# YamaneKoyo/mri-to-speech

Measured on AMD Instinct MI355X. Metric: rtMRI frames/s end-to-end (256x256 frames -> 64-bin mel -> 11413 Hz wav), higher is better.
Workload: dtype bf16x3; 1 GPU; e2e rtMRI->wav, 64 clips x 30 frames per GPU at 256x256 (configs[3] per-GPU share); clips_per_gpu=64, frames_per_clip=30, global_batch_clips=64, hw=256, parallelism=dp1, chunk=1920

## Files before the change

### mri-to-speech_amd/csrc/ir_ws.hip

```cpp
#include <algorithm>
#include <cstdlib>
#include <type_traits>
#include <vector>

#include "kernels.hpp"
#include "lds_dma.hpp"
#include "prof.hpp"

namespace m2s {
namespace {

constexpr int WS_SL = 32;
constexpr int WS_BR = 8;
constexpr int WS_NP = 8;
constexpr int WS_NC = 8;
constexpr int WS_UMAX = 3;

__device__ __forceinline__ int hx_of(int r) { return ((r & 3) << 2) | swz_f((r >> 2) & 3); }

struct WsLayout {
  int XR, TROWS, x_bytes, tile_bytes, w_bytes, total;
};

__host__ __device__ inline int ws_cpp(int cs_in) { return (cs_in * 2 + 255) / 256 * 16; }
// ... 228 lines not shown
      TR(f, 13);
      bump(pdone_p);
      if (JOINT) {
        wait_pd_tf(f, d2);
        return;
      }
      if (f + 1 < T) wait_ge(pdone_p, NPC * (unsigned)(f + 1));
      TR(f, 14);
      if (f + 2 < T) issue_w(f + 2, d2);
    }
  };
  auto produce = [&](int f, Step d, Step d2) {
    const int r0 = d.band * WS_BR, br = min(WS_BR, H - r0), xr0 = max(r0 - 1, 0), xr1 = min(r0 + WS_BR + 1, H);
    const int PB = (xr1 - xr0) * W, nunit = 2 * ((PB + 15) / 16);
    const char* wb = wbuf + (f & 1) * KS * 4096;
    const int hxl = hx_of(r16);
    static_assert(WS_NP % 2 == 0, "unit -> channel tile");
    const int wrow = (wave & 1) * 16 + r16;
    const int wo = wrow * 64 + ((g ^ swz_f((wrow >> 2) & 3)) << 4);
    const int nu = nunit > wave ? (nunit - wave + WS_NP - 1) / WS_NP : 0;
    char* tb = tiles + (f & 1) * 8 * PLT;
    const int trow0 = xr0 - r0 + 1;
    const float4 bb = *reinterpret_cast<const float4*>(bpl + (f & 1) * 32 + (wave & 1) * 16 + 4 * g);
    auto units = [&](auto nuc) {
      constexpr int NU = decltype(nuc)::value;
      f32x4 acc[NU];
#pragma unroll
      for (int k = 0; k < NU; ++k) acc[k] = f32x4{0.f, 0.f, 0.f, 0.f};
      constexpr int D = !IRWS_PF_DEEP ? 2 : NU == 1 ? 4 : NU == 2 ? 3 : 2;
      bf16x8 ah[D], al[D], bh[D][NU], bl[D][NU];
      auto load = [&](int ks, int bsel) {
        const int Lh = ks * 4 + g, Ll = CPP + ks * 4 + g;
        const int ph = ((Lh & ~15) | ((Lh & 15) ^ hxl)) << 4, pl = ((Ll & ~15) | ((Ll & 15) ^ hxl)) << 4;
        ah[bsel] = *reinterpret_cast<const bf16x8*>(wb + ks * 4096 + wo);
        al[bsel] = *reinterpret_cast<const bf16x8*>(wb + ks * 4096 + 2048 + wo);
#pragma unroll
        for (int k = 0; k < NU; ++k) {
          const char* xr = xs + (((wave + WS_NP * k) >> 1) * 16 + r16) * XP;
          bh[bsel][k] = *reinterpret_cast<const bf16x8*>(xr + ph);
          bl[bsel][k] = *reinterpret_cast<const bf16x8*>(xr + pl);
        }
      };
#pragma unroll
      for (int ks = 0; ks < D - 1 && ks < KS; ++ks) load(ks, ks);
#pragma unroll
      for (int ks = 0; ks < KS; ++ks) {
        const int c = ks % D;
        if (ks + D - 1 < KS) load(ks + D - 1, (ks + D - 1) % D);
        __builtin_amdgcn_sched_barrier(0);
#pragma unroll
        for (int k = 0; k < NU; ++k) {
          acc[k] = __builtin_amdgcn_mfma_f32_16x16x32_bf16(al[c], bh[c][k], acc[k], 0, 0, 0);
          acc[k] = __builtin_amdgcn_mfma_f32_16x16x32_bf16(ah[c], bl[c][k], acc[k], 0, 0, 0);
          acc[k] = __builtin_amdgcn_mfma_f32_16x16x32_bf16(ah[c], bh[c][k], acc[k], 0, 0, 0);
        }
      }
      TR(f, 6);
      after_mfma(f, d2);
      TR(f, 8);
      if (!JOINT && f >= 2) wait_all(tfree, (unsigned)(f - 1));
      TR(f, 9);
#pragma unroll
      for (int k = 0; k < NU; ++k) {
        const int u = wave + WS_NP * k, nt = u & 1, m = (u >> 1) * 16 + r16;
        if (m < PB) {
          const int ti = (m / W + trow0) * WT + (m % W) + 1;
          *reinterpret_cast<float4*>(tb + (nt * 4 + g) * PLT + ti * 16) =
              make_float4(silu(acc[k][0] + bb.x), silu(acc[k][1] + bb.y), silu(acc[k][2] + bb.z), silu(acc[k][3] + bb.w));
        }
      }
    };
    static_assert(WS_UMAX == 3, "unit counts 1..3");
    if (nu == 3) units(std::integral_constant<int, 3>());
    else if (nu == 2) units(std::integral_constant<int, 2>());
    else if (nu == 1) units(std::integral_constant<int, 1>());
    else {
      after_mfma(f, d2);
      if (!JOINT && f >= 2) wait_all(tfree, (unsigned)(f - 1));
    }
    if (tid < 8 * W) {
      const int pl = tid / W, c = tid - pl * W;
      const float4 z = make_float4(0.f, 0.f, 0.f, 0.f);
      if (r0 == 0) *reinterpret_cast<float4*>(tb + pl * PLT + (c + 1) * 16) = z;
      if (r0 + br == H) *reinterpret_cast<float4*>(tb + pl * PLT + ((br + 1) * WT + c + 1) * 16) = z;
    }
  };

  const int ct = tid - 64 * WS_NP, cw = ct >> 6, cg = ct & 7, cpl = ct >> 3;
  int cpo = cpl, toff0 = ((cpl / W) * WT + cpl % W) * 16;
  if constexpr (S == 2) {
    const int k = cpl >> 2, i = cpl & 3, c0 = (k >> 1) + 4 * (k & 1);
    const int oy = 2 * (k & 1) + (i & 1), ox = (((i & 1) ? c0 + 6 : c0) + 4 * (i >> 1)) & 7;
    cpo = oy * OWS + ox;
    toff0 = ((2 * oy - pad_t + 1) * WT + 2 * ox - pad_l + 1) * 16;
  }
  auto consume = [&](int f, Step d) {
    const int c0 = d.sl * WS_SL, r0 = d.band * WS_BR, br = min(WS_BR, H - r0);
    float s[4] = {0.f, 0.f, 0.f, 0.f};
    TR(f, 4);
    const uint32_t pbase = (uint32_t)(d.img * PO + (r0 / S) * OWS);
    const uint32_t yoffb = __builtin_amdgcn_readfirstlane(4u * (uint32_t)c0) + (fm32 ? 16u : 8u) * (uint32_t)cg +
                           pbase * (4u * (uint32_t)cs_mid);
    const uint32_t yoff0 = yoffb + (uint32_t)cpo * (4u * (uint32_t)cs_mid);
    const float* wd = wdl + (f % 3) * 320 + 4 * cg;
    float w[9][4], b[4];
#pragma unroll
    for (int t = 0; t < 9; ++t) {
      const float4 v = *reinterpret_cast<const float4*>(wd + t * 32);
      w[t][0] = v.x; w[t][1] = v.y; w[t][2] = v.z; w[t][3] = v.w;
    }
    {
      const float4 v = *reinterpret_cast<const float4*>(wd + 288);
      b[0] = v.x; b[1] = v.y; b[2] = v.z; b[3] = v.w;
    }
    const char* tpl = tiles + (f & 1) * 8 * PLT + cg * PLT;
    auto pixel = [&](int k) {
      const char* tp = tpl + toff0 + k * (64 / W) * WT * 16;
      float a[4] = {b[0], b[1], b[2], b[3]};
#pragma unroll
      for (int t = 0; t < 9; ++t) {
        const float4 u = *reinterpret_cast<const float4*>(tp + ((t / 3) * WT + (t % 3)) * 16);
        a[0] += w[t][0] * u.x;
        a[1] += w[t][1] * u.y;
        a[2] += w[t][2] * u.z;
        a[3] += w[t][3] * u.w;
        if (t == 5) asm volatile("" ::: "memory");
      }
#pragma unroll
      for (int j = 0; j < 4; ++j) {
        a[j] = silu(a[j]);
        s[j] += a[j];
      }
      char* u = reinterpret_cast<char*>(y) + (yoff0 + (uint32_t)k * 256u * (uint32_t)cs_mid);
      if (fm32) {
        *reinterpret_cast<float4*>(u) = make_float4(a[0], a[1], a[2], a[3]);
      } else {
        uint2 hi, lo;
        split4(a, hi, lo);
        *reinterpret_cast<uint2*>(u) = hi;
        *reinterpret_cast<uint2*>(u + 64) = lo;
      }
    };
    auto pixel_pair = [&]() {
      const int pa = cpl >> 4, pc = cpl & 15;
      const char* tp = tpl + ((2 * pa) * WT + pc) * 16;
      float a0[4] = {b[0], b[1], b[2], b[3]}, a1[4] = {b[0], b[1], b[2], b[3]};
#pragma unroll
      for (int ry = 0; ry < 4; ++ry) {
#pragma unroll
        for (int rx = 0; rx < 3; ++rx) {
          const float4 u = *reinterpret_cast<const float4*>(tp + (ry * WT + rx) * 16);
          if (ry < 3) {
            const int t = ry * 3 + rx;
            a0[0] += w[t][0] * u.x; a0[1] += w[t][1] * u.y; a0[2] += w[t][2] * u.z; a0[3] += w[t][3] * u.w;
          }
          if (ry > 0) {
            const int t = (ry - 1) * 3 + rx;
            a1[0] += w[t][0] * u.x; a1[1] += w[t][1] * u.y; a1[2] += w[t][2] * u.z; a1[3] += w[t][3] * u.w;
          }
        }
        if (ry == 1) asm volatile("" ::: "memory");
      }
      const uint32_t po = (uint32_t)(32 * pa + pc);
      auto out = [&](float* a, uint32_t pos) {
#pragma unroll
        for (int j = 0; j < 4; ++j) {
          a[j] = silu(a[j]);
          s[j] += a[j];
        }
        char* u = reinterpret_cast<char*>(y) + (yoffb + pos * (4u * (uint32_t)cs_mid));
        if (fm32) {
          *reinterpret_cast<float4*>(u) = make_float4(a[0], a[1], a[2], a[3]);
        } else {
          uint2 hi, lo;
          split4(a, hi, lo);
          *reinterpret_cast<uint2*>(u) = hi;
          *reinterpret_cast<uint2*>(u + 64) = lo;
        }
      };
      out(a0, po);
      out(a1, po + 16u);
    };
    if constexpr (S == 2) {
      if (cpl < OPB) pixel(0);
    } else if (IRWS_PAIR && W == 16 && br == WS_BR) {
      pixel_pair();
    } else if (br == WS_BR) {
#pragma unroll
      for (int k = 0; k < WS_PXL; ++k) pixel(k);
    } else {
#pragma unroll
      for (int k = 0; k < WS_PXL; ++k)
        if (cpl + 64 * k < br * W) pixel(k);
    }
    TR(f, 5);
    bump(tfree + cw);
    TR(f, 10);
#pragma unroll
    for (int j = 0; j < 4; ++j) {
      s[j] += __builtin_bit_cast(float, __builtin_amdgcn_update_dpp(0, __builtin_bit_cast(int, s[j]), 0x128, 0xF, 0xF, false));
      const auto q = __builtin_amdgcn_permlane16_swap(__float_as_uint(s[j]), __float_as_uint(s[j]), false, false);
      s[j] = __uint_as_float(q[0]) + __uint_as_float(q[1]);
      const auto r = __builtin_amdgcn_permlane32_swap(__float_as_uint(s[j]), __float_as_uint(s[j]), false, false);
      s[j] = __uint_as_float(r[0]) + __uint_as_float(r[1]);
    }
    TR(f, 11);
    const int sc = 4 * (lane & 7) + ((lane >> 3) & 3);
    {
      const int j = (lane >> 3) & 3;
      const float v = j == 0 ? s[0] : j == 1 ? s[1] : j == 2 ? s[2] : s[3];
      if (lane < WS_SL && !(__builtin_fabsf(v) < 2147483648.0f))
        asm volatile("ds_write_b32 %0, %1" ::"v"((uint32_t)(uintptr_t)(sq_nan + d.sl)), "v"(1u) : "memory");
      if (lane < WS_SL)
        __hip_atomic_fetch_add(sq + c0 + sc, (unsigned long long)(long long)(__builtin_fabsf(v) < 2147483648.0f ? v * 4294967296.0f : 0.f),
                               __ATOMIC_RELAXED, __HIP_MEMORY_SCOPE_WORKGROUP);
    }
    unsigned arrived = 0;
    if (lane == 0) arrived = __hip_atomic_fetch_add(sq_n + d.sl, 1u, __ATOMIC_ACQ_REL, __HIP_MEMORY_SCOPE_WORKGROUP);
    if (__builtin_amdgcn_readfirstlane(arrived) == (unsigned)(NB * WS_NC - 1) && lane < WS_SL) {
      const unsigned long long t = __hip_atomic_exchange(sq + c0 + sc, 0ull, __ATOMIC_RELAXED, __HIP_MEMORY_SCOPE_WORKGROUP);
      const float m = __fmaf_rn((float)(unsigned)t, 2.3283064365386963e-10f, (float)(int)(t >> 32)) / (float)PO;
      act_st<sp_t>(reinterpret_cast<sp_t*>(se_mean), d.img, cs_mid, c0 + sc, (*poison || sq_nan[d.sl]) ? __builtin_nanf("") : m);
      if (lane == 0) {
        sq_n[d.sl] = 0u;
        sq_nan[d.sl] = 0u;
      }
    }
  };

  __syncthreads();
  if (prod) {
    __builtin_amdgcn_s_setprio(2);
    Step cur = first_step(blockIdx.x);
    if (T > 0) issue_w(0, cur);
    if (T > 1) issue_w(1, next_step(cur));
    if (TAPS_AHEAD && T > 0 && tap_wave) issue_wd(0, cur);
    if (T > 0) {
      wait_vm_le((T > 1 ? npw : 0) + (TAPS_AHEAD && tap_wave ? 1 : 0));
      bump(wrdy_p);
      if (!HAND_END) wait_ge(wrdy_p, NPC);
    }
    static_assert(4 * KS <= 4 * WS_NP, "pieces per wave");
    int bands = 0;
    for (int i = 0; i < T; ++i) {
      const Step nxt = next_step(cur), nxt2 = next_step(nxt);
      TR(i, 0);
      if (cur.sl == cur.lo) {
        if (i > 0) {
          wait_ge(pdone_p, NPC * (unsigned)i);
          if (par) wait_ge(pw ? ctr + 0 : ctr + 5, NPC * (unsigned)i);
        }
        issue_x(cur.img, cur.band);
        wait_vm<0>();
        bump(xrdy);
        wait_ge(xrdy, (unsigned)(WS_NP * ++bands));
      }
      TR(i, 1);
      if (!TAPS_AHEAD && tap_wave) {
        if (i >= 3) wait_all(tfree, (unsigned)(i - 2));
        issue_wd(i, cur);
      }
      if (HAND_END) wait_ge(wrdy_p, NPC * (unsigned)(i + 1));
      TR(i, 2);
      produce(i, cur, nxt2);
      if (HAND_END) {
        wait_vm<0>();
        asm volatile("s_waitcnt lgkmcnt(0)" ::: "memory");
        if (lane == 0) {
          asm volatile("ds_add_u32 %0, %1" ::"v"((uint32_t)(uintptr_t)wrdy_p), "v"(1u) : "memory");
          asm volatile("ds_add_u32 %0, %1" ::"v"((uint32_t)(uintptr_t)tfull), "v"(1u) : "memory");
        }
        TR(i, 12);
        const bool nw = i + 2 < T, nt = TAPS_AHEAD && tap_wave && i + 1 < T;
        if (nw || nt) {
          wait_ge(pdone_p, NPC * (unsigned)(i + 1));
          if (nw) issue_w(i + 2, nxt2);
          if (nt) issue_wd(i + 1, nxt);
        }
      } else {
        if (tap_wave) {
          const bool nt = TAPS_AHEAD && i + 1 < T;
          if (nt) issue_wd(i + 1, nxt);
          wait_vm_le((i + 2 < T ? npw : 0) + (nt ? 1 : 0));
        }
        bump(tfull);
        TR(i, 12);
      }
      TR(i, 3);
      cur = nxt;
    }
  } else {
    Step cur = first_step(blockIdx.x);
    for (int i = 0; i < T; ++i) {
      wait_ge(tfull, (unsigned)(WS_NP * (i + 1)));
      consume(i, cur);
      TR(i, 7);
      cur = next_step(cur);
    }
  }
}

#include "ir_ws_wave.hpp"

constexpr bool ws_wave_shape(int W, int S) { return W == 16 && S == 1; }
template <int W, int KS, int S>
__global__ void __launch_bounds__(ws_wave_shape(W, S) ? 64 * WV_NW : 64 * (WS_NP + WS_NC), 1)
    ir_ws_kernel(const bf16_t* __restrict__ x, int N, int H, int cs_mid, const bf16_t* __restrict__ wpw,
                 const float* __restrict__ bpw, const float* __restrict__ wdw, const float* __restrict__ bdw,
                 bf16_t* __restrict__ y, bf16_t* __restrict__ se_mean, unsigned long long* __restrict__ trace,
                 unsigned spin_max, unsigned* __restrict__ err, int pad_t, int pad_l, int fm32, int n_full, int parts) {
  if constexpr (ws_wave_shape(W, S)) ir_ws_wave16<KS>(x, N, H, cs_mid, wpw, bpw, wdw, bdw, y, se_mean, fm32, n_full, parts);
  else ir_ws_handoff<W, KS, S>(x, N, H, cs_mid, wpw, bpw, wdw, bdw, y, se_mean, trace, spin_max, err, pad_t, pad_l, fm32, n_full, parts);
}
template <int W, int KS, int S, int HANDOFF>
__global__ void __launch_bounds__(64 * (WS_NP + WS_NC), 1)
    ir_ws_kernel(const bf16_t* __restrict__ x, int N, int H, int cs_mid, const bf16_t* __restrict__ wpw,
                 const float* __restrict__ bpw, const float* __restrict__ wdw, const float* __restrict__ bdw,
                 bf16_t* __restrict__ y, bf16_t* __restrict__ se_mean, unsigned long long* __restrict__ trace,
                 unsigned spin_max, unsigned* __restrict__ err, int pad_t, int pad_l, int fm32, int n_full, int parts) {
  static_assert(HANDOFF == 1, "the handed-off form");
  ir_ws_handoff<W, KS, S>(x, N, H, cs_mid, wpw, bpw, wdw, bdw, y, se_mean, trace, spin_max, err, pad_t, pad_l, fm32, n_full, parts);
}

#ifdef IRWS_TRACE
static void dump_trace(unsigned long long* tr, hipStream_t s, const char* tag) {
  static int calls = 0;
  if (++calls > 40) return;
  std::vector<unsigned long long> h(64 * 2 * 16 * 64);
  M2S_HIP(hipStreamSynchronize(s));
  M2S_HIP(hipMemcpy(h.data(), tr, h.size() * 8, hipMemcpyDeviceToHost));
  auto at = [&](int i, int c, int k, int w = 0) { return (long long)h[((i * 2 + c) * 16 + k) * 64 + w]; };
  fprintf(stderr, "TRACE %s:", tag);
  for (int i = 2; i < 12; ++i)
    fprintf(stderr, " [P x %lld wr %lld mfma %lld tf %lld epi %lld hand %lld | C wait %lld px %lld bump %lld shf %lld at %lld]",
            at(i, 0, 1) - at(i, 0, 0), at(i, 0, 2) - at(i, 0, 1), at(i, 0, 6) - at(i, 0, 2), at(i, 0, 9) - at(i, 0, 6),
            at(i, 0, 12) - at(i, 0, 9), at(i, 0, 3) - at(i, 0, 12), at(i, 1, 4) - at(i - 1, 1, 7), at(i, 1, 5) - at(i, 1, 4),
            at(i, 1, 10) - at(i, 1, 5), at(i, 1, 11) - at(i, 1, 10), at(i, 1, 7) - at(i, 1, 11));
  fprintf(stderr, "\n");
  fprintf(stderr, "TRACEW %s:", tag);
  for (int i = 2; i < 4; ++i) {
    fprintf(stderr, " [s%d", i);
    for (int w = 0; w < 8; ++w) {
      fprintf(stderr, " w%d", w);
      for (int k : {0, 2, 6, 9, 12, 3}) fprintf(stderr, "%c%lld", k ? '/' : ' ', at(i, 0, k, w) - at(i, 0, 0));
    }
    fprintf(stderr, "]");
  }
  fprintf(stderr, "\n");
  fprintf(stderr, "TRACEC %s:", tag);
  for (int i = 4; i < 7; ++i) {
    fprintf(stderr, " [s%d P0 mfma_end %lld vm0 %lld pdone %lld after %lld tf %lld tfull %lld |", i, at(i, 0, 6) - at(i, 0, 0),
            at(i, 0, 13) - at(i, 0, 0), at(i, 0, 14) - at(i, 0, 0), at(i, 0, 8) - at(i, 0, 0), at(i, 0, 9) - at(i, 0, 0),
            at(i, 0, 12) - at(i, 0, 0));
    for (int j = i - 2; j <= i; ++j) {
      fprintf(stderr, " c%d:", j);
      for (int w = 0; w < 8; ++w)
        fprintf(stderr, " %lld/%lld/%lld", at(j, 1, 4, w) - at(i, 0, 0), at(j, 1, 10, w) - at(i, 0, 0), at(j, 1, 7, w) - at(i, 0, 0));
    }
    fprintf(stderr, "]");
  }
  fprintf(stderr, "\n");
  M2S_HIP(hipMemset(tr, 0, h.size() * 8));
}
#endif

}

bool ir_ws_s2_supported(int H, int W, int cs_in, int kp, int cs_mid, int OH, int OW, int pad_t, int pad_l) {
  return H == 16 && W == 16 && OH == 8 && OW == 8 && pad_t >= 0 && pad_t <= 1 && pad_l >= 0 && pad_l <= 1 &&
         ir_ws_supported(H, W, cs_in, kp, cs_mid) && ws_layout(H, W, cs_in, cs_mid, 2).total <= 160 * 1024;
}

bool ir_ws_supported(int H, int W, int cs_in, int kp, int cs_mid) {
  if (!((W == 8 && (kp == 128 || kp == 224)) || (W == 16 && kp == 128)) || H < 1 || H > 64 || cs_in != kp) return false;
  if (cs_mid % WS_SL != 0 || cs_mid < 3 * WS_SL) return false;
  const WsLayout L = ws_layout(H, W, cs_in, cs_mid);
  const int cpr = 2 * ws_cpp(cs_in);
  return L.total <= 160 * 1024 && (L.XR * W * cpr) % 64 == 0 && L.XR * W * cpr / 64 / WS_NP + 1 <= 60 &&
         2 * ((L.XR * W + 15) / 16) <= WS_NP * WS_UMAX;
}

void launch_ir_ws(const void* x, int N, int H, int W, int cs_in, int kp, int cs_mid, const void* wpw, const float* bpw,
                  const float* wdw, const float* bdw, void* y, void* se_mean, double flops, double bytes,
                  hipStream_t s, AsyncReport rep, int stride, int OH, int OW, int pad_t, int pad_l, double spill,
                  bool fm32, int forced_parts, bool handoff) {
  M2S_CHECK(stride == 1 ? ir_ws_supported(H, W, cs_in, kp, cs_mid)
                        : stride == 2 && ir_ws_s2_supported(H, W, cs_in, kp, cs_mid, OH, OW, pad_t, pad_l),
            "ir_ws: unsupported shape");
  M2S_CHECK(N > 0, "ir_ws: no images");
  M2S_CHECK((double)N * H * W * cs_mid * 4.0 < 4294967296.0, "ir_ws: output map too large for 32-bit offsets");
  const WsLayout L = ws_layout(H, W, cs_in, cs_mid, stride);
  const int n_cu = device_cus();
  const dim3 grid(std::min(N, n_cu));
  const int G = (int)grid.x, NSl = cs_mid / WS_SL;
  const int n_full = N / G * G, rem = N - n_full;
  int parts = rem > 0 ? std::max(1, (G + rem / 2) / rem) : 1;
  parts = std::max(1, std::min(parts, NSl / 3));
  if (forced_parts > 0) parts = std::min(forced_parts, std::max(1, NSl / 3));
#ifdef IRWS_TRACE
  static unsigned long long* tr = [] {
    unsigned long long* p = nullptr;
    if (getenv("M2S_IR_WS_TRACE")) M2S_HIP(hipMalloc(&p, 64 * 2 * 16 * 64 * 8));
    return p;
  }();
#define M2S_IRWS_DUMP(tag) \
  if (tr) dump_trace(tr, s, tag);
#else
  unsigned long long* tr = nullptr;
#define M2S_IRWS_DUMP(tag)
#endif
  const bf16_t* xb = static_cast<const bf16_t*>(x);
  const bf16_t* wb = static_cast<const bf16_t*>(wpw);
  bf16_t* yb = static_cast<bf16_t*>(y);
  bf16_t* mb = static_cast<bf16_t*>(se_mean);
  const bool wave_form = ws_wave_shape(W, stride) && H <= 16 && !handoff;
#define M2S_IRWS_GO(KERNEL_, THREADS_, LDS_, NAME_)                                                     \
  {                                                                                                     \
    allow_lds(reinterpret_cast<const void*>(&KERNEL_));                                                 \
    ProfScope ps(NAME_, flops, bytes, s, spill);                                                        \
    hipLaunchKernelGGL((KERNEL_), grid, dim3(THREADS_), LDS_, s, xb, N, H, cs_mid, wb, bpw, wdw, bdw, yb, mb, tr, \
                       rep.spin_max, rep.err, pad_t, pad_l, fm32 ? 1 : 0, n_full, parts);               \
    M2S_IRWS_DUMP(NAME_)                                                                                \
    M2S_HIP(hipGetLastError());                                                                         \
    return;                                                                                             \
  }
  if (ws_wave_shape(W, stride) && kp == 128) {
    if (wave_form) M2S_IRWS_GO((ir_ws_kernel<16, 4, 1>), 64 * WV_NW, WV_NW * 1024 + H * W * 2 * ws_cpp(cs_in) * 16, "ir_ws_kernel<16, 4, 1>")
    M2S_IRWS_GO((ir_ws_kernel<16, 4, 1, 1>), 64 * (WS_NP + WS_NC), L.total, "ir_ws_kernel<16, 4, 1, 1>")
  }
#define M2S_IRWS(W_, KS_, S_, NAME_)                                                                    \
  if (W == W_ && kp == KS_ * 32 && stride == S_) M2S_IRWS_GO((ir_ws_kernel<W_, KS_, S_>), 64 * (WS_NP + WS_NC), L.total, NAME_)
  M2S_IRWS(8, 4, 1, "ir_ws_kernel<8, 4, 1>") M2S_IRWS(8, 7, 1, "ir_ws_kernel<8, 7, 1>")
  M2S_IRWS(16, 4, 2, "ir_ws_kernel<16, 4, 2>")
#undef M2S_IRWS_GO
#undef M2S_IRWS
#undef M2S_IRWS_DUMP
  M2S_CHECK(false, "ir_ws: no variant for this shape");
}

}
```

### mri-to-speech_amd/csrc/ir_ws_wave.hpp

```cpp
#pragma once


#ifndef IRWS_WAVE_ABL
#define IRWS_WAVE_ABL 0
#endif
constexpr int WV_NW = 8;
constexpr int WV_GC = 16;
constexpr int WV_PF = 5;

__device__ __forceinline__ float dpp_left(float v) {
  return __builtin_bit_cast(float, __builtin_amdgcn_update_dpp(0, __builtin_bit_cast(int, v), 0x111, 0xF, 0xF, true));
}
__device__ __forceinline__ float dpp_right(float v) {
  return __builtin_bit_cast(float, __builtin_amdgcn_update_dpp(0, __builtin_bit_cast(int, v), 0x101, 0xF, 0xF, true));
}
template <int ROR>
__device__ __forceinline__ float dpp_ror_add(float v) {
  return v + __builtin_bit_cast(float, __builtin_amdgcn_update_dpp(0, __builtin_bit_cast(int, v), 0x120 + ROR, 0xF, 0xF, false));
}

template <int KS, bool FULL, bool F32>
__device__ __forceinline__ void ir_ws_wave16(const bf16_t* __restrict__ x, int N, int H, int cs_mid,
                                             const bf16_t* __restrict__ wpw, const float* __restrict__ bpw,
                                             const float* __restrict__ wdw, const float* __restrict__ bdw,
                                             bf16_t* __restrict__ y, bf16_t* __restrict__ se_mean, int n_full, int parts) {
  constexpr int W = 16, HMAX = 16;
  constexpr int CS = KS * 32;
  constexpr int CPP = (CS * 2 + 255) / 256 * 16;
  constexpr int CPR = 2 * CPP;
  constexpr int XP = CPR * 16;
  extern __shared__ __attribute__((aligned(16))) char smem[];
  char* xs = smem + WV_NW * 1024;
  const int tid = threadIdx.x, lane = tid & 63;
  const int wave = __builtin_amdgcn_readfirstlane(tid >> 6);
  const int g = lane >> 4, r16 = lane & 15;
  const int NG = cs_mid / WV_GC, P = H * W;
  const int n_units = n_full + (N - n_full) * parts;
  const char* zpage = zero_page();
  const int hxl = hx_of(r16);

  struct AFrag {
    bf16x8 h[KS], l[KS];
  };
  auto lane_now = [&]() {
    int ln = lane;
    asm volatile("" : "+v"(ln));
    return ln;
  };
  auto load_a = [&](int cg) {
    AFrag a;
    const int ln = lane_now();
    const bf16_t* wr = wpw + ((size_t)(cg * WV_GC + (ln & 15)) * CS * 2 + (ln >> 4) * 8);
#pragma unroll
    for (int ks = 0; ks < KS; ++ks) {
      a.h[ks] = *reinterpret_cast<const bf16x8*>(wr + ks * 32);
      a.l[ks] = *reinterpret_cast<const bf16x8*>(wr + CS + ks * 32);
    }
    return a;
  };

  struct Taps {
    float4 w[9], bp, bd;
  };
  char* const tslot = smem + wave * 1024;
  auto issue_taps = [&](int cg) {
    const int ln = lane_now(), t = ln >> 2, c = cg * WV_GC + 4 * (ln & 3);
    const void* src = t < 9 ? static_cast<const void*>(wdw + (t * cs_mid + c))
                            : t == 9 ? static_cast<const void*>(bpw + c) : t == 10 ? static_cast<const void*>(bdw + c) : zpage;
    dma16_asm(src, lds_lo32_u(tslot));
  };
  auto read_taps = [&]() {
    Taps t;
#pragma unroll
    for (int k = 0; k < 9; ++k) t.w[k] = *reinterpret_cast<const float4*>(tslot + k * 64 + g * 16);
    t.bp = *reinterpret_cast<const float4*>(tslot + 9 * 64 + g * 16);
    t.bd = *reinterpret_cast<const float4*>(tslot + 10 * 64 + g * 16);
    return t;
  };

  for (int u = blockIdx.x; u < n_units; u += gridDim.x) {
    int img = u, glo = 0, ghi = NG;
    if (u >= n_full) {
      const int q = u - n_full, pt = q % parts;
      img = n_full + q / parts;
      glo = pt * NG / parts;
      ghi = (pt + 1) * NG / parts;
    }
    int cg = glo + wave;
    AFrag a;
    if (cg < ghi) {
      issue_taps(cg);
      a = load_a(cg);
    }
    __syncthreads();
    if (!(IRWS_WAVE_ABL & 4) || u == (int)blockIdx.x) {
      const int ninstr = P * CPR / 64;
      const bf16_t* xi = x + (size_t)img * P * CS * 2;
      for (int j = wave; j < ninstr; j += WV_NW) {
        const int id = j * 64 + lane, r = id / CPR, p = id - r * CPR;
        const int L = (p & ~15) | ((p & 15) ^ hx_of(r));
        const int plane = L / CPP, k8 = L - plane * CPP;
        const void* src = k8 * 8 < CS ? static_cast<const void*>(xi + (size_t)r * CS * 2 + plane * CS + k8 * 8) : zpage;
        dma16_asm(src, lds_lo32_u(xs + j * 1024));
      }
    }
    __builtin_amdgcn_s_waitcnt(0x0F70);
    asm volatile("" ::: "memory");
    __syncthreads();

    auto unit = [&]() {
      const int c4 = cg * WV_GC + 4 * g;
      f32x4 acc[HMAX];
      {
        constexpr int NI = HMAX * KS;
        bf16x8 bh[WV_PF], bl[WV_PF];
        auto load_b = [&](int i) {
          const int T = i / KS, ks = i % KS;
          const char* xr = xs + (T * 16 + r16) * XP;
          const int Lh = ks * 4 + g, Ll = CPP + ks * 4 + g;
          const int ph = ((Lh & ~15) | ((Lh & 15) ^ hxl)) << 4, pl = ((Ll & ~15) | ((Ll & 15) ^ hxl)) << 4;
          bh[i % WV_PF] = *reinterpret_cast<const bf16x8*>(xr + ph);
          bl[i % WV_PF] = *reinterpret_cast<const bf16x8*>(xr + pl);
        };
#pragma unroll
        for (int i = 0; i < WV_PF - 1; ++i)
          if (FULL || i / KS < H) load_b(i);
#pragma unroll
        for (int i = 0; i < NI; ++i) {
          const int T = i / KS, ks = i % KS, ip = i + WV_PF - 1;
          if (FULL || T < H) {
            if (ip < NI && (FULL || ip / KS < H)) load_b(ip);
            __builtin_amdgcn_sched_barrier(0);
            f32x4 c = ks == 0 ? f32x4{0.f, 0.f, 0.f, 0.f} : acc[T];
            c = __builtin_amdgcn_mfma_f32_16x16x32_bf16(a.l[ks], bh[i % WV_PF], c, 0, 0, 0);
            c = __builtin_amdgcn_mfma_f32_16x16x32_bf16(a.h[ks], bl[i % WV_PF], c, 0, 0, 0);
            c = __builtin_amdgcn_mfma_f32_16x16x32_bf16(a.h[ks], bh[i % WV_PF], c, 0, 0, 0);
            acc[T] = c;
          }
        }
      }
      __builtin_amdgcn_sched_barrier(0);
      asm volatile("" ::: "memory");
      const Taps tp = read_taps();
      asm volatile("s_waitcnt lgkmcnt(0)" ::: "memory");
      const int cgn = cg + WV_NW < ghi ? cg + WV_NW : cg;
      issue_taps(cgn);
      const AFrag an = load_a(cgn);
      __builtin_amdgcn_sched_barrier(0);

      const uint32_t ps = 4u * (uint32_t)cs_mid;
      const int lny = lane_now();
      const uint32_t ylane = (uint32_t)(lny & 15) * ps + (F32 ? 4u * (uint32_t)(cg * WV_GC + 4 * (lny >> 4))
                                                              : 128u * (uint32_t)(cg >> 1) + 8u * (uint32_t)((cg & 1) * 4 + (lny >> 4)));
      char* const yimg = reinterpret_cast<char*>(y) + (uint32_t)(img * P) * ps;
      float sum[4] = {0.f, 0.f, 0.f, 0.f};
      const float bbv[4] = {tp.bp.x, tp.bp.y, tp.bp.z, tp.bp.w}, bdv[4] = {tp.bd.x, tp.bd.y, tp.bd.z, tp.bd.w};
      float w[9][4];
#pragma unroll
      for (int t = 0; t < 9; ++t) {
        w[t][0] = tp.w[t].x; w[t][1] = tp.w[t].y; w[t][2] = tp.w[t].z; w[t][3] = tp.w[t].w;
      }
      float prv[4] = {0.f, 0.f, 0.f, 0.f}, cur[4] = {bdv[0], bdv[1], bdv[2], bdv[3]}, nxt[4] = {0.f, 0.f, 0.f, 0.f};
#pragma unroll
      for (int s = 0; s <= HMAX; ++s) {
        if ((IRWS_WAVE_ABL & 2) && s < HMAX && (FULL || s < H)) {
#pragma unroll
          for (int j = 0; j < 4; ++j) nxt[j] = silu(acc[s][j] + bbv[j]) + w[4][j];
        } else if (s < HMAX && (FULL || s < H)) {
#pragma unroll
          for (int j = 0; j < 4; ++j) {
            const float uc = silu(acc[s][j] + bbv[j]);
            const float ul = dpp_left(uc), ur = dpp_right(uc);
            nxt[j] = bdv[j];
            nxt[j] += w[0][j] * ul;
            nxt[j] += w[1][j] * uc;
            nxt[j] += w[2][j] * ur;
            cur[j] += w[3][j] * ul;
            cur[j] += w[4][j] * uc;
            cur[j] += w[5][j] * ur;
            if (s > 0) {
              prv[j] += w[6][j] * ul;
              prv[j] += w[7][j] * uc;
              prv[j] += w[8][j] * ur;
            }
          }
        }
        if (s >= 1 && (FULL || s - 1 < H)) {
          float o[4];
#pragma unroll
          for (int j = 0; j < 4; ++j) {
            o[j] = silu(prv[j]);
            sum[j] += o[j];
          }
          char* dst = yimg + ((uint32_t)(s - 1) * 16u * ps + ylane);
          if (IRWS_WAVE_ABL & 1) {
          } else if (F32) {
            *reinterpret_cast<float4*>(dst) = make_float4(o[0], o[1], o[2], o[3]);
          } else {
            uint2 hi, lo;
            split4(o, hi, lo);
            *reinterpret_cast<uint2*>(dst) = hi;
            *reinterpret_cast<uint2*>(dst + 64) = lo;
          }
        }
#pragma unroll
        for (int j = 0; j < 4; ++j) {
          prv[j] = cur[j];
          cur[j] = nxt[j];
        }
        __builtin_amdgcn_sched_barrier(0);
      }

#pragma unroll
      for (int j = 0; j < 4; ++j) sum[j] = dpp_ror_add<1>(dpp_ror_add<2>(dpp_ror_add<4>(dpp_ror_add<8>(sum[j]))));
      if (r16 < 4) {
        const float v = r16 == 0 ? sum[0] : r16 == 1 ? sum[1] : r16 == 2 ? sum[2] : sum[3];
        act_st<sp_t>(reinterpret_cast<sp_t*>(se_mean), img, cs_mid, c4 + r16, v / (float)P);
      }
      a = an;
    };
    for (; cg < ghi; cg += WV_NW) unit();
  }
}

template <int KS>
__device__ __forceinline__ void ir_ws_wave16(const bf16_t* __restrict__ x, int N, int H, int cs_mid,
                                             const bf16_t* __restrict__ wpw, const float* __restrict__ bpw,
                                             const float* __restrict__ wdw, const float* __restrict__ bdw,
                                             bf16_t* __restrict__ y, bf16_t* __restrict__ se_mean, int fm32, int n_full,
                                             int parts) {
  const bool full = H == 16;
  if (full && fm32) ir_ws_wave16<KS, true, true>(x, N, H, cs_mid, wpw, bpw, wdw, bdw, y, se_mean, n_full, parts);
  else if (full) ir_ws_wave16<KS, true, false>(x, N, H, cs_mid, wpw, bpw, wdw, bdw, y, se_mean, n_full, parts);
  else if (fm32) ir_ws_wave16<KS, false, true>(x, N, H, cs_mid, wpw, bpw, wdw, bdw, y, se_mean, n_full, parts);
  else ir_ws_wave16<KS, false, false>(x, N, H, cs_mid, wpw, bpw, wdw, bdw, y, se_mean, n_full, parts);
}
```

Baseline: 53900 rtMRI frames/s.

## Add wave-specialized 8x8 inverted-residual kernel with double-buffered input prefetch

New measurement: 56250 rtMRI frames/s (median of 6 runs). 1.04x the previous value.

```diff
diff --git a/mri-to-speech_amd/csrc/ir_ws.hip b/mri-to-speech_amd/csrc/ir_ws.hip
--- a/mri-to-speech_amd/csrc/ir_ws.hip
+++ b/mri-to-speech_amd/csrc/ir_ws.hip
@@ -554,14 +554,19 @@
 
 #include "ir_ws_wave.hpp"
 
-constexpr bool ws_wave_shape(int W, int S) { return W == 16 && S == 1; }
+constexpr bool ws_wave_shape(int W, int S) { return (W == 16 || W == 8) && S == 1; }
+constexpr bool ws_wave_height(int W, int H) { return W == 16 ? H <= 16 : H == 8; }
+inline int ws_wave_lds(int H, int W, int cs_in) {
+  return WV_NW * (W == 16 ? 1 : WV8_TS) * 1024 + (W == 16 ? H : 2 * H) * W * 2 * ws_cpp(cs_in) * 16;
+}
 template <int W, int KS, int S>
 __global__ void __launch_bounds__(ws_wave_shape(W, S) ? 64 * WV_NW : 64 * (WS_NP + WS_NC), 1)
     ir_ws_kernel(const bf16_t* __restrict__ x, int N, int H, int cs_mid, const bf16_t* __restrict__ wpw,
                  const float* __restrict__ bpw, const float* __restrict__ wdw, const float* __restrict__ bdw,
                  bf16_t* __restrict__ y, bf16_t* __restrict__ se_mean, unsigned long long* __restrict__ trace,
                  unsigned spin_max, unsigned* __restrict__ err, int pad_t, int pad_l, int fm32, int n_full, int parts) {
-  if constexpr (ws_wave_shape(W, S)) ir_ws_wave16<KS>(x, N, H, cs_mid, wpw, bpw, wdw, bdw, y, se_mean, fm32, n_full, parts);
+  if constexpr (ws_wave_shape(W, S) && W == 16) ir_ws_wave16<KS>(x, N, H, cs_mid, wpw, bpw, wdw, bdw, y, se_mean, fm32, n_full, parts);
+  else if constexpr (ws_wave_shape(W, S)) ir_ws_wave8<KS>(x, N, cs_mid, wpw, bpw, wdw, bdw, y, se_mean, fm32, n_full, parts);
   else ir_ws_handoff<W, KS, S>(x, N, H, cs_mid, wpw, bpw, wdw, bdw, y, se_mean, trace, spin_max, err, pad_t, pad_l, fm32, n_full, parts);
 }
 template <int W, int KS, int S, int HANDOFF>
@@ -665,7 +670,8 @@
   const bf16_t* wb = static_cast<const bf16_t*>(wpw);
   bf16_t* yb = static_cast<bf16_t*>(y);
   bf16_t* mb = static_cast<bf16_t*>(se_mean);
-  const bool wave_form = ws_wave_shape(W, stride) && H <= 16 && !handoff;
+  const bool wave_form = ws_wave_shape(W, stride) && ws_wave_height(W, H) && !handoff;
+  const int wave_lds = ws_wave_lds(H, W, cs_in);
 #define M2S_IRWS_GO(KERNEL_, THREADS_, LDS_, NAME_)                                                     \
   {                                                                                                     \
     allow_lds(reinterpret_cast<const void*>(&KERNEL_));                                                 \
@@ -676,16 +682,20 @@
     M2S_HIP(hipGetLastError());                                                                         \
     return;                                                                                             \
   }
-  if (ws_wave_shape(W, stride) && kp == 128) {
-    if (wave_form) M2S_IRWS_GO((ir_ws_kernel<16, 4, 1>), 64 * WV_NW, WV_NW * 1024 + H * W * 2 * ws_cpp(cs_in) * 16, "ir_ws_kernel<16, 4, 1>")
+  if (W == 16 && stride == 1 && kp == 128) {
+    if (wave_form) M2S_IRWS_GO((ir_ws_kernel<16, 4, 1>), 64 * WV_NW, wave_lds, "ir_ws_kernel<16, 4, 1>")
     M2S_IRWS_GO((ir_ws_kernel<16, 4, 1, 1>), 64 * (WS_NP + WS_NC), L.total, "ir_ws_kernel<16, 4, 1, 1>")
   }
-#define M2S_IRWS(W_, KS_, S_, NAME_)                                                                    \
-  if (W == W_ && kp == KS_ * 32 && stride == S_) M2S_IRWS_GO((ir_ws_kernel<W_, KS_, S_>), 64 * (WS_NP + WS_NC), L.total, NAME_)
-  M2S_IRWS(8, 4, 1, "ir_ws_kernel<8, 4, 1>") M2S_IRWS(8, 7, 1, "ir_ws_kernel<8, 7, 1>")
-  M2S_IRWS(16, 4, 2, "ir_ws_kernel<16, 4, 2>")
+#define M2S_IRWS8(KS_, NAME_)                                                                           \
+  if (W == 8 && kp == KS_ * 32 && stride == 1) {                                                        \
+    if (wave_form) M2S_IRWS_GO((ir_ws_kernel<8, KS_, 1>), 64 * WV_NW, wave_lds, NAME_)                  \
+    if (H == 8) M2S_IRWS_GO((ir_ws_kernel<8, KS_, 1, 1>), 64 * (WS_NP + WS_NC), L.total, "ir_ws_kernel<8, " #KS_ ", 1, 1>") \
+    M2S_IRWS_GO((ir_ws_kernel<8, KS_, 1, 1>), 64 * (WS_NP + WS_NC), L.total, NAME_)                     \
+  }
+  M2S_IRWS8(4, "ir_ws_kernel<8, 4, 1>") M2S_IRWS8(7, "ir_ws_kernel<8, 7, 1>")
+  if (W == 16 && kp == 128 && stride == 2) M2S_IRWS_GO((ir_ws_kernel<16, 4, 2>), 64 * (WS_NP + WS_NC), L.total, "ir_ws_kernel<16, 4, 2>")
 #undef M2S_IRWS_GO
-#undef M2S_IRWS
+#undef M2S_IRWS8
 #undef M2S_IRWS_DUMP
   M2S_CHECK(false, "ir_ws: no variant for this shape");
 }
diff --git a/mri-to-speech_amd/csrc/ir_ws_wave.hpp b/mri-to-speech_amd/csrc/ir_ws_wave.hpp
--- a/mri-to-speech_amd/csrc/ir_ws_wave.hpp
+++ b/mri-to-speech_amd/csrc/ir_ws_wave.hpp
@@ -14,9 +14,57 @@
 __device__ __forceinline__ float dpp_right(float v) {
   return __builtin_bit_cast(float, __builtin_amdgcn_update_dpp(0, __builtin_bit_cast(int, v), 0x101, 0xF, 0xF, true));
 }
+struct WvUnit {
+  int img, glo, ghi;
+};
+__device__ __forceinline__ WvUnit wv_unit_of(int u, int n_full, int parts, int NG) {
+  if (u < n_full) return WvUnit{u, 0, NG};
+  const int q = u - n_full, pt = q % parts;
+  return WvUnit{n_full + q / parts, pt * NG / parts, (pt + 1) * NG / parts};
+}
 template <int ROR>
 __device__ __forceinline__ float dpp_ror_add(float v) {
   return v + __builtin_bit_cast(float, __builtin_amdgcn_update_dpp(0, __builtin_bit_cast(int, v), 0x120 + ROR, 0xF, 0xF, false));
+}
+
+template <int KS>
+struct WvAFrag {
+  bf16x8 h[KS], l[KS];
+};
+__device__ __forceinline__ int wv_lane_now(int lane) {
+  asm volatile("" : "+v"(lane));
+  return lane;
+}
+template <int KS>
+__device__ __forceinline__ WvAFrag<KS> wv_load_a(const bf16_t* __restrict__ wpw, int cg, int ln) {
+  constexpr int CS = KS * 32;
+  WvAFrag<KS> a;
+  const bf16_t* wr = wpw + ((size_t)(cg * WV_GC + (ln & 15)) * CS * 2 + (ln >> 4) * 8);
+#pragma unroll
+  for (int ks = 0; ks < KS; ++ks) {
+    a.h[ks] = *reinterpret_cast<const bf16x8*>(wr + ks * 32);
+    a.l[ks] = *reinterpret_cast<const bf16x8*>(wr + CS + ks * 32);
+  }
+  return a;
+}
+struct WvTaps {
+  float4 w[9], bp, bd;
+};
+__device__ __forceinline__ void wv_issue_taps(const float* __restrict__ wdw, const float* __restrict__ bpw,
+                                              const float* __restrict__ bdw, const char* zpage, int cs_mid, int cg, int ln,
+                                              char* tslot) {
+  const int t = ln >> 2, c = cg * WV_GC + 4 * (ln & 3);
+  const void* src = t < 9 ? static_cast<const void*>(wdw + (t * cs_mid + c))
+                          : t == 9 ? static_cast<const void*>(bpw + c) : t == 10 ? static_cast<const void*>(bdw + c) : zpage;
+  dma16_asm(src, lds_lo32_u(tslot));
+}
+__device__ __forceinline__ WvTaps wv_read_taps(const char* tslot, int g) {
+  WvTaps t;
+#pragma unroll
+  for (int k = 0; k < 9; ++k) t.w[k] = *reinterpret_cast<const float4*>(tslot + k * 64 + g * 16);
+  t.bp = *reinterpret_cast<const float4*>(tslot + 9 * 64 + g * 16);
+  t.bd = *reinterpret_cast<const float4*>(tslot + 10 * 64 + g * 16);
+  return t;
 }
 
 template <int KS, bool FULL, bool F32>
@@ -39,54 +87,18 @@
   const char* zpage = zero_page();
   const int hxl = hx_of(r16);
 
-  struct AFrag {
-    bf16x8 h[KS], l[KS];
-  };
-  auto lane_now = [&]() {
-    int ln = lane;
-    asm volatile("" : "+v"(ln));
-    return ln;
-  };
-  auto load_a = [&](int cg) {
-    AFrag a;
-    const int ln = lane_now();
-    const bf16_t* wr = wpw + ((size_t)(cg * WV_GC + (ln & 15)) * CS * 2 + (ln >> 4) * 8);
-#pragma unroll
-    for (int ks = 0; ks < KS; ++ks) {
-      a.h[ks] = *reinterpret_cast<const bf16x8*>(wr + ks * 32);
-      a.l[ks] = *reinterpret_cast<const bf16x8*>(wr + CS + ks * 32);
-    }
-    return a;
-  };
-
-  struct Taps {
-    float4 w[9], bp, bd;
-  };
+  using AFrag = WvAFrag<KS>;
+  using Taps = WvTaps;
   char* const tslot = smem + wave * 1024;
-  auto issue_taps = [&](int cg) {
-    const int ln = lane_now(), t = ln >> 2, c = cg * WV_GC + 4 * (ln & 3);
-    const void* src = t < 9 ? static_cast<const void*>(wdw + (t * cs_mid + c))
-                            : t == 9 ? static_cast<const void*>(bpw + c) : t == 10 ? static_cast<const void*>(bdw + c) : zpage;
-    dma16_asm(src, lds_lo32_u(tslot));
-  };
-  auto read_taps = [&]() {
-    Taps t;
-#pragma unroll
-    for (int k = 0; k < 9; ++k) t.w[k] = *reinterpret_cast<const float4*>(tslot + k * 64 + g * 16);
-    t.bp = *reinterpret_cast<const float4*>(tslot + 9 * 64 + g * 16);
-    t.bd = *reinterpret_cast<const float4*>(tslot + 10 * 64 + g * 16);
-    return t;
-  };
+  auto lane_now = [&]() { return wv_lane_now(lane); };
+  auto load_a = [&](int cg) { return wv_load_a<KS>(wpw, cg, lane_now()); };
+  auto issue_taps = [&](int cg) { wv_issue_taps(wdw, bpw, bdw, zpage, cs_mid, cg, lane_now(), tslot); };
+  auto read_taps = [&]() { return wv_read_taps(tslot, g); };
 
   for (int u = blockIdx.x; u < n_units; u += gridDim.x) {
-    int img = u, glo = 0, ghi = NG;
-    if (u >= n_full) {
-      const int q = u - n_full, pt = q % parts;
-      img = n_full + q / parts;
-      glo = pt * NG / parts;
-      ghi = (pt + 1) * NG / parts;
-    }
-    int cg = glo + wave;
+    const WvUnit un = wv_unit_of(u, n_full, parts, NG);
+    const int img = un.img, ghi = un.ghi;
+    int cg = un.glo + wave;
     AFrag a;
     if (cg < ghi) {
       issue_taps(cg);
@@ -235,3 +247,227 @@
   else if (fm32) ir_ws_wave16<KS, false, true>(x, N, H, cs_mid, wpw, bpw, wdw, bdw, y, se_mean, n_full, parts);
   else ir_ws_wave16<KS, false, false>(x, N, H, cs_mid, wpw, bpw, wdw, bdw, y, se_mean, n_full, parts);
 }
+
+__device__ __forceinline__ float dpp_swap8(float v) {
+  return __builtin_bit_cast(float, __builtin_amdgcn_update_dpp(0, __builtin_bit_cast(int, v), 0x128, 0xF, 0xF, false));
+}
+
+#ifndef IRWS_WAVE8_G
+#define IRWS_WAVE8_G 1
+#endif
+constexpr int WV8_G = IRWS_WAVE8_G;
+constexpr int WV8_TS = WV8_G == 1 ? 1 : 2 * WV8_G;
+
+template <int KS, bool F32>
+__device__ __forceinline__ void ir_ws_wave8(const bf16_t* __restrict__ x, int N, int cs_mid, const bf16_t* __restrict__ wpw,
+                                            const float* __restrict__ bpw, const float* __restrict__ wdw,
+                                            const float* __restrict__ bdw, bf16_t* __restrict__ y,
+                                            bf16_t* __restrict__ se_mean, int n_full, int parts) {
+  constexpr int NT = 4, P = 64;
+  constexpr int CS = KS * 32;
+  constexpr int CPP = (CS * 2 + 255) / 256 * 16;
+  constexpr int CPR = 2 * CPP;
+  constexpr int XP = CPR * 16;
+  constexpr int XB = P * XP;
+  extern __shared__ __attribute__((aligned(16))) char smem[];
+  char* const xs0 = smem + WV_NW * WV8_TS * 1024;
+  const int tid = threadIdx.x, lane = tid & 63;
+  const int wave = __builtin_amdgcn_readfirstlane(tid >> 6);
+  const int g = lane >> 4, r16 = lane & 15;
+  const int NG = cs_mid / WV_GC;
+  const int n_units = n_full + (N - n_full) * parts;
+  const char* zpage = zero_page();
+  const int hxl = hx_of(r16);
+
+  using AFrag = WvAFrag<KS>;
+  constexpr int G = WV8_G;
+  auto tslot = [&](int q, int par) { return smem + (wave * WV8_TS + (G == 1 ? 0 : par * G + q)) * 1024; };
+  auto lane_now = [&]() { return wv_lane_now(lane); };
+  auto load_a = [&](int cg) { return wv_load_a<KS>(wpw, cg, lane_now()); };
+  auto issue_taps = [&](int cg, char* slot) { wv_issue_taps(wdw, bpw, bdw, zpage, cs_mid, cg, lane_now(), slot); };
+  auto issue_x = [&](int img, char* dst) {
+    constexpr int ninstr = P * CPR / 64;
+    const bf16_t* xi = x + (size_t)img * P * CS * 2;
+    for (int j = wave; j < ninstr; j += WV_NW) {
+      const int id = j * 64 + lane, r = id / CPR, p = id - r * CPR;
+      const int L = (p & ~15) | ((p & 15) ^ hx_of(r));
+      const int plane = L / CPP, k8 = L - plane * CPP;
+      const void* src = k8 * 8 < CS ? static_cast<const void*>(xi + (size_t)r * CS * 2 + plane * CS + k8 * 8) : zpage;
+      dma16_asm(src, lds_lo32_u(dst + j * 1024));
+    }
+  };
+
+  int u = blockIdx.x, buf = 0, par = 0;
+  if (u < n_units) issue_x(wv_unit_of(u, n_full, parts, NG).img, xs0);
+  for (; u < n_units; u += gridDim.x, buf ^= 1) {
+    const WvUnit un = wv_unit_of(u, n_full, parts, NG);
+    const int img = un.img, ghi = un.ghi;
+    int cg = un.glo + G * wave;
+    auto gq = [&](int c, int q) { return c + q < ghi ? c + q : ghi - 1; };
+    AFrag a[G];
+    if (cg < ghi) {
+#pragma unroll
+      for (int q = 0; q < G; ++q) {
+        issue_taps(gq(cg, q), tslot(q, par));
+        a[q] = load_a(gq(cg, q));
+      }
+    }
+    __builtin_amdgcn_s_waitcnt(0x0F70);
+    asm volatile("" ::: "memory");
+    __syncthreads();
+    const int u_next = u + (int)gridDim.x;
+    if (u_next < n_units && !(IRWS_WAVE_ABL & 4)) issue_x(wv_unit_of(u_next, n_full, parts, NG).img, xs0 + (buf ^ 1) * XB);
+    const char* const xs = xs0 + ((IRWS_WAVE_ABL & 4) ? 0 : buf * XB);
+
+    auto unit = [&]() {
+      f32x4 acc[G][NT];
+      {
+        constexpr int NI = NT * KS;
+        bf16x8 bh[WV_PF], bl[WV_PF];
+        auto load_b = [&](int i) {
+          const int T = i / KS, ks = i % KS;
+          const char* xr = xs + (T * 16 + r16) * XP;
+          const int Lh = ks * 4 + g, Ll = CPP + ks * 4 + g;
+          const int ph = ((Lh & ~15) | ((Lh & 15) ^ hxl)) << 4, pl = ((Ll & ~15) | ((Ll & 15) ^ hxl)) << 4;
+          bh[i % WV_PF] = *reinterpret_cast<const bf16x8*>(xr + ph);
+          bl[i % WV_PF] = *reinterpret_cast<const bf16x8*>(xr + pl);
+        };
+#pragma unroll
+        for (int i = 0; i < WV_PF - 1; ++i) load_b(i);
+#pragma unroll
+        for (int i = 0; i < NI; ++i) {
+          const int T = i / KS, ks = i % KS, ip = i + WV_PF - 1;
+          if (ip < NI) load_b(ip);
+          __builtin_amdgcn_sched_barrier(0);
+#pragma unroll
+          for (int q = 0; q < G; ++q) {
+            f32x4 c = ks == 0 ? f32x4{0.f, 0.f, 0.f, 0.f} : acc[q][T];
+            c = __builtin_amdgcn_mfma_f32_16x16x32_bf16(a[q].l[ks], bh[i % WV_PF], c, 0, 0, 0);
+            c = __builtin_amdgcn_mfma_f32_16x16x32_bf16(a[q].h[ks], bl[i % WV_PF], c, 0, 0, 0);
+            c = __builtin_amdgcn_mfma_f32_16x16x32_bf16(a[q].h[ks], bh[i % WV_PF], c, 0, 0, 0);
+            acc[q][T] = c;
+          }
+        }
+      }
+      __builtin_amdgcn_sched_barrier(0);
+      asm volatile("" ::: "memory");
+      WvTaps tp0;
+      if (G == 1) {
+        tp0 = wv_read_taps(tslot(0, 0), g);
+        asm volatile("s_waitcnt lgkmcnt(0)" ::: "memory");
+      }
+      const int cgn = cg + G * WV_NW < ghi ? cg + G * WV_NW : cg;
+      AFrag an[G];
+#pragma unroll
+      for (int q = 0; q < G; ++q) {
+        issue_taps(gq(cgn, q), tslot(q, par ^ 1));
+        an[q] = load_a(gq(cgn, q));
+      }
+      __builtin_amdgcn_sched_barrier(0);
+
+      auto depthwise = [&](const f32x4 (&acc)[NT], const WvTaps& tp, int cg) {
+      const int c4 = cg * WV_GC + 4 * g;
+      const uint32_t ps = 4u * (uint32_t)cs_mid;
+      const int lny = lane_now();
+      const uint32_t ylane = (uint32_t)(lny & 15) * ps + (F32 ? 4u * (uint32_t)(cg * WV_GC + 4 * (lny >> 4))
+                                                              : 128u * (uint32_t)(cg >> 1) + 8u * (uint32_t)((cg & 1) * 4 + (lny >> 4)));
+      char* const yimg = reinterpret_cast<char*>(y) + (uint32_t)(img * P) * ps;
+      const bool col0 = (lny & 7) == 0, col7 = (lny & 7) == 7, half = (lny & 8) != 0;
+      float sum[4] = {0.f, 0.f, 0.f, 0.f};
+      const float bbv[4] = {tp.bp.x, tp.bp.y, tp.bp.z, tp.bp.w}, bdv[4] = {tp.bd.x, tp.bd.y, tp.bd.z, tp.bd.w};
+      float w[9][4];
+#pragma unroll
+      for (int t = 0; t < 9; ++t) {
+        w[t][0] = tp.w[t].x; w[t][1] = tp.w[t].y; w[t][2] = tp.w[t].z; w[t][3] = tp.w[t].w;
+      }
+      float cur[4] = {0.f, 0.f, 0.f, 0.f}, vprev[4] = {0.f, 0.f, 0.f, 0.f};
+#pragma unroll
+      for (int s = 0; s <= NT; ++s) {
+        float o[4];
+#pragma unroll
+        for (int j = 0; j < 4; ++j) {
+          if (IRWS_WAVE_ABL & 2) {
+            if (s >= 1) o[j] = silu(acc[s - 1][j] + bbv[j]) + w[4][j];
+            continue;
+          }
+          float uc = 0.f, ul = 0.f, ur = 0.f, v = 0.f;
+          if (s < NT) {
+            uc = silu(acc[s][j] + bbv[j]);
+            const float ml = dpp_left(uc), mr = dpp_right(uc);
+            ul = col0 ? 0.f : ml;
+            ur = col7 ? 0.f : mr;
+            v = dpp_swap8(uc);
+          }
+          const float up = half ? v : vprev[j];
+          const float mul = dpp_left(up), mur = dpp_right(up);
+          const float upl = col0 ? 0.f : mul, upr = col7 ? 0.f : mur;
+          vprev[j] = v;
+          if (s >= 1) {
+            float c = cur[j];
+            c += w[6][j] * upl;
+            c += w[7][j] * up;
+            c += w[8][j] * upr;
+            o[j] = c;
+          }
+          if (s < NT) {
+            float n = bdv[j];
+            n += w[0][j] * upl;
+            n += w[1][j] * up;
+            n += w[2][j] * upr;
+            n += w[3][j] * ul;
+            n += w[4][j] * uc;
+            n += w[5][j] * ur;
+            cur[j] = n;
+          }
+        }
+        if (s >= 1) {
+#pragma unroll
+          for (int j = 0; j < 4; ++j) {
+            o[j] = silu(o[j]);
+            sum[j] += o[j];
+          }
+          char* dst = yimg + ((uint32_t)(s - 1) * 16u * ps + ylane);
+          if (IRWS_WAVE_ABL & 1) {
+          } else if (F32) {
+            *reinterpret_cast<float4*>(dst) = make_float4(o[0], o[1], o[2], o[3]);
+          } else {
+            uint2 hi, lo;
+            split4(o, hi, lo);
+            *reinterpret_cast<uint2*>(dst) = hi;
+            *reinterpret_cast<uint2*>(dst + 64) = lo;
+          }
+        }
+        __builtin_amdgcn_sched_barrier(0);
+      }
+
+#pragma unroll
+      for (int j = 0; j < 4; ++j) sum[j] = dpp_ror_add<1>(dpp_ror_add<2>(dpp_ror_add<4>(dpp_ror_add<8>(sum[j]))));
+      if (r16 < 4) {
+        const float v = r16 == 0 ? sum[0] : r16 == 1 ? sum[1] : r16 == 2 ? sum[2] : sum[3];
+        act_st<sp_t>(reinterpret_cast<sp_t*>(se_mean), img, cs_mid, c4 + r16, v / (float)P);
+      }
+      };
+#pragma unroll
+      for (int q = 0; q < G; ++q) {
+        if (G == 1) {
+          depthwise(acc[q], tp0, cg);
+        } else {
+          const WvTaps tp = wv_read_taps(tslot(q, par), g);
+          depthwise(acc[q], tp, gq(cg, q));
+        }
+        a[q] = an[q];
+      }
+      if (G > 1) par ^= 1;
+    };
+    for (; cg < ghi; cg += G * WV_NW) unit();
+  }
+}
+
+template <int KS>
+__device__ __forceinline__ void ir_ws_wave8(const bf16_t* __restrict__ x, int N, int cs_mid, const bf16_t* __restrict__ wpw,
+                                            const float* __restrict__ bpw, const float* __restrict__ wdw,
+                                            const float* __restrict__ bdw, bf16_t* __restrict__ y,
+                                            bf16_t* __restrict__ se_mean, int fm32, int n_full, int parts) {
+  if (fm32) ir_ws_wave8<KS, true>(x, N, cs_mid, wpw, bpw, wdw, bdw, y, se_mean, n_full, parts);
+  else ir_ws_wave8<KS, false>(x, N, cs_mid, wpw, bpw, wdw, bdw, y, se_mean, n_full, parts);
+}
```
